# huzaifakhan04/truely-real-time-ai-generated-video-detection-framework-for-social-platforms

Hardware: AMD Instinct MI355X
Metric: frames/sec (detect+embed+drift) 720p (higher is better)
Workload: dtype f32; 1 GPU; BASELINE configs[1]: synthetic 720p 1-face frames, batch=256 per GPU, fp32, MTCNN detect + 80x80 crop + InceptionResnetV1 embed + cosine drift score; frames_per_gpu=256, height=720, width=1280, weights=seeded synthetic (no checkpoints offline), prelu_slopes=unit, min_face_size=20, pyramid_levels=11, valid_faces=256, score=6, emb_crc32=3015932725, mode=sharded, ingest=resident, parallelism=single GPU, batches_in_flight=1, driver=single, embed_group=8

## Files before the change

### truely-real-time-ai-generated-video-detection-framework-for-social-platforms_amd/csrc/trl_api.hip

```cpp
#include <limits.h>
#include <stdarg.h>
#include <stdio.h>
#include <string.h>
#include <stdlib.h>

#include "trl_ctx.h"

static thread_local char g_err[512] = "";
int g_trl_no_fnconv = 0;
int g_trl_pnet_gate = 0;

#include <mutex>
namespace {
std::mutex g_gate_mu;
hipEvent_t g_gate_ev[64] = {};
bool g_gate_set[64] = {};
}
int trl_gate_wait(trl_ctx* c, hipStream_t s) {
    const int d = c->cfg.device;
    if (!g_trl_pnet_gate || d < 0 || d >= 64) return TRL_OK;
    std::lock_guard<std::mutex> lk(g_gate_mu);
    if (g_gate_set[d]) TRL_HIP(hipStreamWaitEvent(s, g_gate_ev[d], 0));
    return TRL_OK;
}
// ... 856 lines not shown
    TRL_CHECK(check_crop_hook(c, d_frames, n, 65535, H, W, d_rect, d_valid, S, d_faces));
    return trl_launch_crop_area_std(d_frames, n, H, W, d_rect, d_valid, S, rgb != 0, d_faces, (hipStream_t)stream);
}
int trl_debug_nms_tiers(trl_ctx* c, int small_tier, int full_tier) {
    TRL_CHECK(trl_check_idle(c));
    if ((small_tier && (small_tier < 16 || small_tier > 3072 || (small_tier & 3))) || (full_tier && (full_tier < 16 || full_tier > 3072 || (full_tier & 3)))) {
        trl_set_error("tiers must be multiples of 4 in [16, 3072]");
        return TRL_ERR_INVALID;
    }
    if (small_tier) c->nms_small = small_tier;
    if (full_tier) c->nms_full = full_tier;
    return TRL_OK;
}
int trl_debug_list_stats(trl_ctx* c, long long* h_out8) {
    if (!c || !h_out8) { trl_set_error("null argument"); return TRL_ERR_INVALID; }
    const int32_t* f = c->h_pinned + 4;
    unsigned long long used = 0;
    memcpy(&used, f + FLG_SPILL_CUR, 8);
    int mx = 0;
    for (int l = 0; l < 32; l++) if (f[FLG_LEVEL_MAX + l] > mx) mx = f[FLG_LEVEL_MAX + l];
    h_out8[0] = c->last_attempts; h_out8[1] = f[FLG_SPILL_LISTS]; h_out8[2] = (long long)used; h_out8[3] = (long long)c->cb.spill_cap;
    h_out8[4] = c->cb.capF; h_out8[5] = c->cb.lay.S; h_out8[6] = mx; h_out8[7] = f[FLG_FRAME_MAX];
    return TRL_OK;
}

int trl_debug_option(trl_ctx* c, const char* key, int value) {
    if (!key) { trl_set_error("null key"); return TRL_ERR_INVALID; }
    if (!strcmp(key, "no_fnconv")) { g_trl_no_fnconv = value ? 1 : 0; return TRL_OK; }
    if (!strcmp(key, "pnet_gate")) { g_trl_pnet_gate = value ? 1 : 0; return TRL_OK; }
    TRL_CHECK(trl_check_idle(c));
    if (!strcmp(key, "rnet_chunk") && value >= 16) { c->rnet_chunk = value; return TRL_OK; }
    if (!strcmp(key, "onet_chunk") && value >= 16) { c->onet_chunk = value; return TRL_OK; }
    if (!strcmp(key, "pnet_screen") && (value == 0 || value == 1)) { c->pnet_screen = value; return TRL_OK; }
    trl_set_error("unknown option '%s' (or value %d out of range)", key, value);
    return TRL_ERR_INVALID;
}

int trl_debug_pnet_screen_bound(trl_ctx* c, float* A, float* B, int* on) {
    if (!c || !A || !B || !on) { trl_set_error("null argument"); return TRL_ERR_INVALID; }
    *A = c->pnet_scrA; *B = c->pnet_scrB; *on = c->pnet_screen_ok && c->pnet_screen;
    return TRL_OK;
}

int trl_debug_batch_capacity(trl_ctx* c, float t2_per_frame, float t3_per_frame, int* last_attempts) {
    if (!c) { trl_set_error("null context"); return TRL_ERR_INVALID; }
    if (t2_per_frame > 0.f) c->t2_per_frame = t2_per_frame;
    if (t3_per_frame > 0.f) c->t3_per_frame = t3_per_frame;
    if (last_attempts) *last_attempts = c->last_attempts;
    return TRL_OK;
}

int trl_debug_stage_totals(trl_ctx* c, int32_t* h_out2) {
    if (!c || !h_out2) { trl_set_error("null argument"); return TRL_ERR_INVALID; }
    h_out2[0] = c->h_pinned[4 + FLG_T2N]; h_out2[1] = c->h_pinned[4 + FLG_T3N];
    return TRL_OK;
}

int trl_debug_pnet_run(trl_ctx* c, int run) {
    if (!c || run < 0 || run > 64) { trl_set_error("bad argument"); return TRL_ERR_INVALID; }
    c->pnet_run = run;
    return TRL_OK;
}

int trl_debug_pnet_span(trl_ctx* c, int reset, double* ms_sum, int32_t* launches) {
    if (!c || !ms_sum || !launches) { trl_set_error("null argument"); return TRL_ERR_INVALID; }
    *ms_sum = 0.0; *launches = 0;
// ... 28 lines not shown
```

### truely-real-time-ai-generated-video-detection-framework-for-social-platforms_amd/csrc/trl_ctx.h

```cpp
#pragma once
#include "trl_common.h"

struct Cand {
    float x1, y1, x2, y2, score;
    float r0, r1, r2, r3;
    int cell;
};

struct LevelGeom {
    double scale;
    int h, w;
    int oh, ow;
};

struct LvLayout {
    int L = 0, S = 0;
    int capl[32] = {0}, rec0[32] = {0};
};
struct CascadeBufs {
    int n = 0, L = 0, H = 0, W = 0;
    LvLayout lay;
    int capF = 0;
    int32_t* lvl_cnt = nullptr;
    Cand* lvl_rec = nullptr;
// ... 33 lines not shown
    float last_ms[4] = {0, 0, 0, 0};
    int pnet_mono1 = 0;
    int pnet_unit = 0;
    float pnet_scrA = 0.f, pnet_scrB = 0.f;
    int pnet_screen_ok = 0;
    int pnet_screen = 1;
    int pnet_run = 0;
    int32_t* pnet_cursor = nullptr;
    unsigned long long* pnet_clk = nullptr;
    bool pnet_prof = false;
    float pnet_kernel_ms = 0.f;
    int dbg_poison = -1;
    float t2_per_frame = 160.f, t3_per_frame = 48.f;
    int cap_t2 = 0, cap_t3 = 0;
    float lvl_hint[32] = {0}, frame_hint = 0.f;
    size_t spill_hint = 0;
    int rnet_chunk = 49152, onet_chunk = 16384;
    int nms_small = 512, nms_full = 2048;
    int last_attempts = 0;
    int resume_stage = 0;
    size_t scratch_after_cascade = 0;
    int rnet_front_mode = -1, onet_front_mode = -1;
    struct Pending {
        enum Kind { EMBED, CROP, DETECT };
        bool active = false; int attempt = 0; Kind kind = EMBED;
        const uint8_t* frames = nullptr; int n = 0, H = 0, W = 0;
        void* stream = nullptr;
        float* box = nullptr; float* prob = nullptr; int32_t* rect = nullptr; uint8_t* valid = nullptr; float* emb = nullptr;
        float* faces_out = nullptr;
        float* boxes = nullptr; float* probs = nullptr; float* points = nullptr; int32_t* counts = nullptr; int order = 0;
    } pend;
    uint32_t* pyr_tab = nullptr;
    int pyr_tab_H = 0, pyr_tab_W = 0;
    struct { int nlev = 0, own0 = 0, band_cols = 0, strip_rows = 0, n_bands = 0, n_strips = 0; } pyr_fine;
    struct { int L = 0; int32_t row[16][TRL_PYR_PLAN_COLS] = {}; } pyr_plan;
    std::vector<trl_fn_plan_row> fn_plan;
    std::vector<trl_fn_plan_row> mt_plan;
    bool mt_plan_arm = false;
    int fn_cap_arm = -1;
    struct { void* p = nullptr; size_t cap = 0; int32_t dims[5] = {0, 0, 0, 0, 0}; } fn_cap[3];
};

struct TrlConvChoice { int family = 0, bm = 0, bn = 0, bk = 0, pad = 0, nz = 1; };
extern thread_local TrlConvChoice g_trl_conv_choice;

int trl_gate_wait(trl_ctx* c, hipStream_t s);
int trl_gate_record(trl_ctx* c, hipStream_t s);
extern int g_trl_pnet_gate;
int trl_ensure(trl_ctx* c, Arena& a, size_t bytes);
int trl_check_idle(trl_ctx* c);
const DevW* trl_w(trl_ctx* c, const std::string& name);
const DevV* trl_v(trl_ctx* c, const std::string& name);

int trl_run_facenet(trl_ctx* c, const float* d_faces, int n, int h, int w, const uint8_t* d_valid, float* d_emb, hipStream_t s);
int trl_run_rnet(trl_ctx* c, const float* d_crops, int n, float* d_out6, hipStream_t s);
int trl_run_onet(trl_ctx* c, const float* d_crops, int n, float* d_out16, hipStream_t s);
int trl_run_rnet_tail(trl_ctx* c, const float* d_pool1, int n, float* d_out6, hipStream_t s, const int32_t* n_dev = nullptr, int n_base = 0);
int trl_run_onet_tail(trl_ctx* c, const float* d_pool1, int n, float* d_out16, hipStream_t s, const int32_t* n_dev = nullptr, int n_base = 0);
int trl_launch_rnet_front(trl_ctx* c, const uint8_t* d_frames, int H, int W, const int32_t* d_total, int t0, int nc, float* d_pool, hipStream_t s);
int trl_launch_onet_front(trl_ctx* c, const uint8_t* d_frames, int H, int W, const int32_t* d_total, int t0, int nc, float* d_pool, hipStream_t s);
int trl_stage_net(trl_ctx* c, int net, const uint8_t* d_frames, int H, int W, const int32_t* d_total, int cap, float* d_out, hipStream_t s);
int trl_run_pnet_generic(trl_ctx* c, const float* d_level, int nf, int h, int w, float* d_heads, hipStream_t s);
size_t trl_pnet_generic_bytes(int nf, int h, int w);

int trl_cascade_detect(trl_ctx* c, const uint8_t* d_frames, int n, int H, int W, hipStream_t s, int resume = 0);
int trl_cascade_finish(trl_ctx* c, const uint8_t* d_frames, int n, int H, int W, float* d_boxes, float* d_probs, float* d_points,
// ... 24 lines not shown
```

### truely-real-time-ai-generated-video-detection-framework-for-social-platforms_amd/csrc/trl_pyramid.hip

```cpp
#include "trl_pyramid.h"
#include <type_traits>

typedef unsigned u32x4_a4 __attribute__((ext_vector_type(4), aligned(4)));
struct __attribute__((packed, aligned(4))) u32x3_a4 { unsigned x, y, z; };

namespace {

__device__ __forceinline__ void dword_sums(unsigned v, int rel, int nbytes, unsigned& s0, unsigned& s1, unsigned& s2) {
    const int lo = rel < 0 ? -rel : 0;
    const int hi = (nbytes - rel) < 4 ? (nbytes - rel) : 4;
    const unsigned vm = (hi >= 4 ? 0xFFFFFFFFu : ((1u << (8 * hi)) - 1u)) & ~((1u << (8 * lo)) - 1u);
    v &= vm;
    const int phase = (rel + 3) % 3;
    const unsigned m0 = phase == 0 ? 0x01000001u : (phase == 1 ? 0x00010000u : 0x00000100u);
    const unsigned m1 = phase == 0 ? 0x00000100u : (phase == 1 ? 0x01000001u : 0x00010000u);
    const unsigned m2 = phase == 0 ? 0x00010000u : (phase == 1 ? 0x00000100u : 0x01000001u);
    s0 = __builtin_amdgcn_udot4(v, m0, s0, false);
    s1 = __builtin_amdgcn_udot4(v, m1, s1, false);
    s2 = __builtin_amdgcn_udot4(v, m2, s2, false);
}

__device__ __forceinline__ unsigned chan_mask(int p, int c) {
    const int d = (c - p + 3) % 3;
    return d == 0 ? 0x01000001u : (d == 1 ? 0x00000100u : 0x00010000u);
}
__device__ __forceinline__ unsigned valid_bytes(int rel, int nbytes) {
    const int lo = rel < 0 ? -rel : 0;
    int hi = nbytes - rel; hi = hi < 0 ? 0 : (hi > 4 ? 4 : hi);
    if (lo >= hi) return 0u;
    return (hi >= 4 ? 0xFFFFFFFFu : ((1u << (8 * hi)) - 1u)) & ~((1u << (8 * lo)) - 1u);
}

typedef float f32x4_nt __attribute__((ext_vector_type(4)));
__device__ __forceinline__ void pyr_store(PyrPx* dst, const float4& v) {
    static_assert(sizeof(PyrPx) == 12, "layout");
    f32x3_nt t = {v.x, v.y, v.z};
    __builtin_nontemporal_store(t, reinterpret_cast<f32x3_nt*>(dst));
}

__device__ __forceinline__ float pyr_div(float a, float b, float r) {
    const float q0 = a * r;
    const float e = __builtin_fmaf(-b, q0, a);
    return __builtin_fmaf(e, r, q0);
}
__device__ __forceinline__ float pyr_norm(unsigned s, int kh, int kw, const PyrBins& g) {
    const float a = (float)s, fkh = (float)kh, fkw = (float)kw;
    float q;
    if (g.fastdiv) {
        const float r1 = kh == g.khA ? g.rkh[0] : g.rkh[1], r2 = kw == g.kwA ? g.rkw[0] : g.rkw[1];
        q = pyr_div(pyr_div(a, fkh, r1), fkw, r2);
    } else {
        q = a / fkh / fkw;
    }
    return (q - 127.5f) * 0.0078125f;
}

struct PyrArgs { int H, W, n_frames, f0; long long pyr_stride; PyrLevel g; };

template <int MODE>
__device__ __forceinline__ void pyr_level(const uint8_t* __restrict__ frames, const PyrArgs& a, const PyrLevel& g, const uint32_t* __restrict__ tab,
                                          PyrPx* __restrict__ pyr, int f, int q0, int qstep) {
    const int per_frame = g.pix_pad << g.gshift;
    constexpr int mode = MODE;
    const uint32_t* base32 = reinterpret_cast<const uint32_t*>(frames);
    const long long fbase = (long long)f * a.H * a.W * 3;
    const long long last_dw = ((long long)a.n_frames * a.H * a.W * 3 - 1) >> 2;
    const int row_bytes = a.W * 3;
    for (int q = q0; q < per_frame; q += qstep) {
        const int w = g.w, gsh = g.gshift, G = 1 << gsh;
        const int pixel = q >> gsh, sub = q & (G - 1);
        const bool valid = pixel < g.h * w;
        unsigned s0 = 0, s1 = 0, s2 = 0;
        int kh = 1, kw = 1;
        if (valid) {
            int oy = (int)__umulhi((unsigned)pixel, g.wmagic);
            oy -= (oy * w > pixel) ? 1 : 0;
// ... 274 lines not shown
                        c0 = n0; c1 = n1; c2 = n2; n0 = 0; n1 = 0; n2 = 0;
                        oy++;
                        ys_c = ys_n; ye_c = ye_n;
                        edges(oy + 1, ys_n, ye_n);
                    }
                }
            }
        }
    };
    if (lastf && yend >= a.H) run(std::true_type{}); else run(std::false_type{});
}

__global__ __launch_bounds__(192) void k_pyramid_fine(const uint8_t* __restrict__ frames, PyrFineArgs a, const uint32_t* __restrict__ tab,
                                                      PyrPx* __restrict__ pyr) {
    const int lane = threadIdx.x & 63, lvl = __builtin_amdgcn_readfirstlane((int)threadIdx.x >> 6);
    if (lvl >= a.nlev) return;
    const int band = blockIdx.x, strip = blockIdx.z, f = blockIdx.y;
    const uint32_t* own = tab + a.own0;
    const uint32_t cb = own[lvl * a.n_bands + band], rb = own[3 * a.n_bands + lvl * a.n_strips + strip];
    const int ox_lo = __builtin_amdgcn_readfirstlane((int)(cb & 0xFFFF)), ox_hi = __builtin_amdgcn_readfirstlane((int)(cb >> 16));
    const int oy_lo = __builtin_amdgcn_readfirstlane((int)(rb & 0xFFFF)), oy_hi = __builtin_amdgcn_readfirstlane((int)(rb >> 16));
    const bool pad_wave = band == 0 && strip == 0;
    if (lvl == 0) { if (a.g[0].kwmax * 3 + 3 > 16) pyr_fine_wave<true>(frames, a, a.g[0], tab, pyr, f, ox_lo, ox_hi, oy_lo, oy_hi, lane, pad_wave); else pyr_fine_wave<false>(frames, a, a.g[0], tab, pyr, f, ox_lo, ox_hi, oy_lo, oy_hi, lane, pad_wave); }
    else if (lvl == 1) { if (a.g[1].kwmax * 3 + 3 > 16) pyr_fine_wave<true>(frames, a, a.g[1], tab, pyr, f, ox_lo, ox_hi, oy_lo, oy_hi, lane, pad_wave); else pyr_fine_wave<false>(frames, a, a.g[1], tab, pyr, f, ox_lo, ox_hi, oy_lo, oy_hi, lane, pad_wave); }
    else { if (a.g[2].kwmax * 3 + 3 > 16) pyr_fine_wave<true>(frames, a, a.g[2], tab, pyr, f, ox_lo, ox_hi, oy_lo, oy_hi, lane, pad_wave); else pyr_fine_wave<false>(frames, a, a.g[2], tab, pyr, f, ox_lo, ox_hi, oy_lo, oy_hi, lane, pad_wave); }
}

constexpr int SMAXL = 12;
constexpr int SBYTES = 4096;
constexpr int SW_BYTES = 1280;
constexpr int STAB = 6144;
struct PyrStreamArgs {
    int H, W, n_frames, nlev, rows_per_band, cols_per_band, row_bands, col_bands;
    long long pyr_stride;
    PyrBins lv[SMAXL];
};

struct OwnBlock {
    static constexpr int LANES = 256, DW = 4, UNITS = 1, BYTES = SBYTES;
    static __device__ __forceinline__ int lane() { return threadIdx.x; }
    static __device__ __forceinline__ int slot() { return 0; }
    static __device__ __forceinline__ void sync() { __syncthreads(); }
    static __device__ __forceinline__ int uni(int x) { return x; }
};
struct OwnWave {
    static constexpr int LANES = 64, DW = 5, UNITS = 4, BYTES = SW_BYTES;
    static __device__ __forceinline__ int lane() { return threadIdx.x & 63; }
    static __device__ __forceinline__ int slot() { return __builtin_amdgcn_readfirstlane((int)threadIdx.x >> 6); }
    static __device__ __forceinline__ void sync() { __builtin_amdgcn_wave_barrier(); }
    static __device__ __forceinline__ int uni(int x) { return __builtin_amdgcn_readfirstlane(x); }
};

template <int NL, class Own>
__global__ __launch_bounds__(256) void k_pyramid_stream(const uint8_t* __restrict__ frames, PyrStreamArgs a, const uint32_t* __restrict__ gtab,
                                                        PyrPx* __restrict__ pyr) {
    constexpr int DW = Own::DW, LANES = Own::LANES;
    static_assert(Own::BYTES == 4 * DW * LANES && Own::UNITS * LANES == 256, "a lane's dwords tile the segment, the units the workgroup");
    __shared__ unsigned colbuf_all[Own::UNITS * Own::BYTES];
    __shared__ uint32_t tab[STAB];
    const int tid = threadIdx.x, lane = Own::lane(), slot = Own::slot();
    const int f = blockIdx.y;
    const int row_bytes = a.W * 3;
    const long long fbase = (long long)f * a.H * row_bytes;
    const long long last_dw = ((long long)a.n_frames * a.H * row_bytes - 1) >> 2;
    const uint32_t* base32 = reinterpret_cast<const uint32_t*>(frames);
    int ty0[NL], tx0[NL];
    {
        int pos = 0;
#pragma unroll
        for (int l = 0; l < NL; l++) {
            ty0[l] = tx0[l] = 0;
            if (l < a.nlev) {
                const PyrBins& g = a.lv[l];
                ty0[l] = pos; tx0[l] = pos + g.h;
                for (int i = tid; i < g.h; i += 256) tab[pos + i] = gtab[g.ytab0 + i];
                for (int i = tid; i < g.w; i += 256) tab[pos + g.h + i] = gtab[g.xtab0 + i];
                pos += g.h + g.w;
            }
        }
    }
    __syncthreads();
    const int unit = blockIdx.x * Own::UNITS + slot;
    if (Own::UNITS > 1 && unit >= a.row_bands * a.col_bands) return;
    const int rb = unit / a.col_bands, cb = unit - rb * a.col_bands;
    const int R0 = rb * a.rows_per_band, R1 = (R0 + a.rows_per_band < a.H) ? R0 + a.rows_per_band : a.H;
    const int C0 = cb * a.cols_per_band, C1 = (C0 + a.cols_per_band < a.W) ? C0 + a.cols_per_band : a.W;
    unsigned* colbuf = colbuf_all + slot * Own::BYTES;

    int j[NL], jend[NL], ys[NL], ye[NL], ox0[NL], ox1[NL];
    int yend = R0;
#pragma unroll
    for (int l = 0; l < NL; l++) {
        j[l] = jend[l] = 0; ys[l] = ye[l] = 0x7fffffff; ox0[l] = ox1[l] = 0;
        if (l < a.nlev) {
            const PyrBins& g = a.lv[l];
            auto first_at_or_after = [&](int tab0, int n_out, int n_in, int pos) {
                if (pos >= n_in) return n_out;
                int q = (int)(((long long)pos * n_out + n_in - 1) / n_in);
                if (q > n_out) q = n_out;
                while (q > 0 && (int)(tab[tab0 + q - 1] & 0xFFFF) >= pos) q--;
                while (q < n_out && (int)(tab[tab0 + q] & 0xFFFF) < pos) q++;
                return q;
            };
            j[l] = Own::uni(first_at_or_after(ty0[l], g.h, a.H, R0));
            jend[l] = Own::uni(first_at_or_after(ty0[l], g.h, a.H, R1));
            ox0[l] = Own::uni(first_at_or_after(tx0[l], g.w, a.W, C0));
            ox1[l] = Own::uni(first_at_or_after(tx0[l], g.w, a.W, C1));
            if (j[l] < jend[l] && ox0[l] < ox1[l]) {
                const uint32_t t0 = tab[ty0[l] + j[l]], t1 = tab[ty0[l] + jend[l] - 1];
                ys[l] = Own::uni((int)(t0 & 0xFFFF)); ye[l] = Own::uni((int)(t0 >> 16));
                const int e1 = Own::uni((int)(t1 >> 16));
                yend = e1 > yend ? e1 : yend;
            } else {
                j[l] = jend[l];
            }
        }
    }
    if (unit == 0) {
#pragma unroll
        for (int l = 0; l < NL; l++)
            if (l < a.nlev) {
                const PyrBins& g = a.lv[l];
                for (int p = g.h * g.w + lane; p < g.pix_pad; p += LANES)
                    pyr_store(pyr + ((long long)f * a.pyr_stride + g.pix0 + p), make_float4(0.f, 0.f, 0.f, 0.f));
            }
    }
    if (yend <= R0) return;

    unsigned ev[NL][DW], od[NL][DW];
#pragma unroll
    for (int l = 0; l < NL; l++)
#pragma unroll
        for (int d = 0; d < DW; d++) { ev[l][d] = 0; od[l][d] = 0; }

    auto load_row = [&](int y, unsigned (&w)[DW + 1], unsigned& sh) {
        const int yy = y < a.H ? y : a.H - 1;
        const long long o = fbase + (long long)yy * row_bytes + (long long)C0 * 3;
        sh = (unsigned)(o & 3);
        const long long dw = (o >> 2) + DW * lane;
        if (dw + DW <= last_dw) {
            const u32x4_a4 v4 = *reinterpret_cast<const u32x4_a4*>(base32 + dw);
            w[0] = v4[0]; w[1] = v4[1]; w[2] = v4[2]; w[3] = v4[3];
#pragma unroll
            for (int k = 4; k <= DW; k++) w[k] = base32[dw + k];
        } else {
#pragma unroll
            for (int k = 0; k <= DW; k++) w[k] = base32[dw + k <= last_dw ? dw + k : last_dw];
        }
    };
    auto consume = [&](int y, const unsigned (&w)[DW + 1], unsigned sh) {
        unsigned v[DW];
#pragma unroll
        for (int d = 0; d < DW; d++) v[d] = __builtin_amdgcn_alignbyte(w[d + 1], w[d], sh);
#pragma unroll
        for (int l = 0; l < NL; l++) {
            if (l < a.nlev && y >= ys[l] && y < ye[l]) {
#pragma unroll
                for (int d = 0; d < DW; d++) { ev[l][d] += v[d] & 0x00FF00FFu; od[l][d] += (v[d] >> 8) & 0x00FF00FFu; }
                if (y == ye[l] - 1) {
                    const PyrBins& g = a.lv[l];
                    const int kh = ye[l] - ys[l];
#pragma unroll
                    for (int d = 0; d < DW; d++) {
                        colbuf[4 * DW * lane + 4 * d + 0] = ev[l][d] & 0xFFFFu; colbuf[4 * DW * lane + 4 * d + 1] = od[l][d] & 0xFFFFu;
                        colbuf[4 * DW * lane + 4 * d + 2] = ev[l][d] >> 16;     colbuf[4 * DW * lane + 4 * d + 3] = od[l][d] >> 16;
                    }
                    Own::sync();
                    for (int ox = ox0[l] + lane; ox < ox1[l]; ox += LANES) {
                        const uint32_t tx = tab[tx0[l] + ox];
                        const int xs = tx & 0xFFFF, xe = tx >> 16;
                        unsigned s0 = 0, s1 = 0, s2 = 0;
                        for (int xx = xs; xx < xe; xx++) {
                            const unsigned* p = colbuf + (xx - C0) * 3;
                            s0 += p[0]; s1 += p[1]; s2 += p[2];
                        }
                        float4 o4;
                        o4.x = pyr_norm(s0, kh, xe - xs, g); o4.y = pyr_norm(s1, kh, xe - xs, g); o4.z = pyr_norm(s2, kh, xe - xs, g);
                        o4.w = 0.f;
                        pyr_store(pyr + ((long long)f * a.pyr_stride + g.pix0 + (long long)j[l] * g.w + ox), o4);
                    }
                    Own::sync();
                    j[l]++;
                    if (j[l] < jend[l]) {
                        const uint32_t t0 = tab[ty0[l] + j[l]];
                        ys[l] = Own::uni((int)(t0 & 0xFFFF)); ye[l] = Own::uni((int)(t0 >> 16));
                    } else {
                        ys[l] = ye[l] = 0x7fffffff;
                    }
                    const bool again = ys[l] <= y;
#pragma unroll
                    for (int d = 0; d < DW; d++) {
                        ev[l][d] = again ? (v[d] & 0x00FF00FFu) : 0u;
                        od[l][d] = again ? ((v[d] >> 8) & 0x00FF00FFu) : 0u;
                    }
                }
            }
        }
    };

    unsigned wb[4][DW + 1], shb[4];
#pragma unroll
    for (int u = 0; u < 4; u++) load_row(R0 + u, wb[u], shb[u]);
    for (int y = R0; y < yend; y += 4) {
#pragma unroll
        for (int u = 0; u < 4; u++) {
            unsigned wc[DW + 1];
#pragma unroll
            for (int k = 0; k <= DW; k++) wc[k] = wb[u][k];
            const unsigned shc = shb[u];
            if (y + u + 4 < yend) load_row(y + u + 4, wb[u], shb[u]);
            if (y + u < yend) consume(y + u, wc, shc);
        }
    }
}

}

int trl_pyramid_layout(trl_ctx* c, int H, int W, PyrLayout& lay) {
    const int L = trl_compute_levels(c, H, W);
    if (L > 16) { trl_set_error("more than 16 pyramid levels"); return TRL_ERR_INVALID; }
    if (L < 1) { trl_set_error("frame %dx%d has no pyramid level at min_face_size %d", W, H, c->cfg.min_face_size); return TRL_ERR_INVALID; }
    lay.L = L;
    int ntab = 0; long long pix = 0;
    for (int l = 0; l < L; l++) {
        const LevelGeom& g = c->lv[l];
        PyrLevel& p = lay.lv[l];
        p.h = g.h; p.w = g.w;
        p.pix0 = (int)pix;
        p.pix_pad = (int)(((long long)g.h * g.w + 63) & ~63ll);
        pix += p.pix_pad;
        const int khmax = (H + g.h - 1) / g.h + 1, kwmax = (W + g.w - 1) / g.w + 1;
        p.khA = (H + g.h - 1) / g.h; p.kwA = (W + g.w - 1) / g.w;
        p.khmax = (H % g.h) ? p.khA + 1 : p.khA; p.kwmax = (W % g.w) ? p.kwA + 1 : p.kwA;
        p.rkh[0] = 1.0f / (float)p.khA; p.rkh[1] = 1.0f / (float)(p.khA + 1);
        p.rkw[0] = 1.0f / (float)p.kwA; p.rkw[1] = 1.0f / (float)(p.kwA + 1);
        p.fastdiv = (p.khA + 1 <= 96 && p.kwA + 1 <= 96) ? 1 : 0;
        for (int d = 0; d < 4; d++) {
            auto vb = [](int rel, int nbytes) { int hi = nbytes - rel; hi = hi < 0 ? 0 : (hi > 4 ? 4 : hi); return hi >= 4 ? 0xFFFFFFFFu : ((1u << (8 * hi)) - 1u); };
            p.vmA[d] = vb(4 * d, 3 * p.kwA); p.vmB[d] = vb(4 * d, 3 * (p.kwA + 1));
        }
        p.wmagic = (unsigned)((0x100000000ull + g.w - 1) / g.w);
        p.hmagic = (unsigned)((0x100000000ull + g.h - 1) / g.h);
        p.arith = ((unsigned long long)(H + 1) * g.h * g.h < 0x100000000ull && (unsigned long long)(W + 1) * g.w * g.w < 0x100000000ull &&
                   g.h > 1 && g.w > 1) ? 1 : 0;
// ... 58 lines not shown
static int pyr_tables(trl_ctx* c, int H, int W, const PyrLayout& lay, hipStream_t s) {
    if (c->pyr_tab != nullptr && c->pyr_tab_H == H && c->pyr_tab_W == W) return TRL_OK;
    std::vector<uint32_t> tab;
    for (int l = 0; l < lay.L; l++) {
        const PyrLevel& g = lay.lv[l];
        for (int i = 0; i < g.h; i++) tab.push_back((uint32_t)(((long long)i * H) / g.h) | ((uint32_t)((((long long)i + 1) * H + g.h - 1) / g.h) << 16));
        for (int i = 0; i < g.w; i++) tab.push_back((uint32_t)(((long long)i * W) / g.w) | ((uint32_t)((((long long)i + 1) * W + g.w - 1) / g.w) << 16));
    }
    pyr_fine_ownership(c, H, W, lay, tab);
    TRL_HIP(hipStreamSynchronize(s));
    if (c->pyr_tab) TRL_HIP(hipFree(c->pyr_tab));
    c->pyr_tab = nullptr;
    TRL_HIP(hipMalloc((void**)&c->pyr_tab, tab.size() * 4 + 64));
    TRL_HIP(hipMemcpy(c->pyr_tab, tab.data(), tab.size() * 4, hipMemcpyHostToDevice));
    c->pyr_tab_H = H; c->pyr_tab_W = W;
    return TRL_OK;
}

struct PyrJob { trl_ctx* c; const uint8_t* frames; int n, H, W; const PyrLayout& lay; PyrPx* pyr; hipStream_t s; };
static void plan_row(const PyrJob& j, int l, int kind, int rb, int cb, int cpb, int frames) {
    int32_t* r = j.c->pyr_plan.row[l];
    r[0] = kind; r[1] = rb; r[2] = cb; r[3] = cpb; r[4] = frames; r[5] = j.lay.lv[l].khmax;
}

static int launch_coarse(const PyrJob& j, bool (&taken)[16]) {
    const int n = j.n, H = j.H, W = j.W;
    int lv_idx[16], nsel = 0;
    for (int l = 0; l < j.lay.L; l++) if (j.lay.lv[l].mode != 0) lv_idx[nsel++] = l;
    const bool wide = W * 3 > SBYTES;
    for (int g0 = 0; g0 < nsel; g0 += 8) {
        const int gn = nsel - g0 < 8 ? nsel - g0 : 8;
        PyrStreamArgs sa;
        sa.nlev = 0;
        int stab_words = 0, kwm = 0;
        bool ok = true;
        for (int q = 0; q < gn; q++) {
            const PyrLevel& g = j.lay.lv[lv_idx[g0 + q]];
            if (g.khmax > 256) ok = false;
            stab_words += g.h + g.w;
            kwm = g.kwmax > kwm ? g.kwmax : kwm;
            sa.lv[sa.nlev++] = g;
        }
        sa.H = H; sa.W = W; sa.n_frames = n; sa.pyr_stride = j.lay.pyr_stride;
        sa.row_bands = H >= 256 ? 3 : 1;
        sa.rows_per_band = (H + sa.row_bands - 1) / sa.row_bands;
        if (!ok || stab_words > STAB || n > 65535) continue;
        if (!wide) {
            if ((kwm + 2) * 3 > SBYTES / 2) continue;
            sa.col_bands = 1; sa.cols_per_band = W;
            const dim3 sgrid(sa.row_bands * sa.col_bands, n);
            if (sa.nlev <= 4) k_pyramid_stream<4, OwnBlock><<<sgrid, 256, 0, j.s>>>(j.frames, sa, j.c->pyr_tab, j.pyr);
            else k_pyramid_stream<8, OwnBlock><<<sgrid, 256, 0, j.s>>>(j.frames, sa, j.c->pyr_tab, j.pyr);
        } else {
            sa.cols_per_band = SW_BYTES / 3 - kwm;
            if (sa.cols_per_band < 64) continue;
            sa.col_bands = (W + sa.cols_per_band - 1) / sa.cols_per_band;
            sa.cols_per_band = (W + sa.col_bands - 1) / sa.col_bands;
            int rbn = (4096 + n * sa.col_bands - 1) / (n * sa.col_bands);
            if (rbn > H / 256) rbn = H / 256;
            if (rbn > sa.row_bands) { sa.row_bands = rbn; sa.rows_per_band = (H + rbn - 1) / rbn; }
            const dim3 sgrid((sa.row_bands * sa.col_bands + 3) / 4, n);
            if (sa.nlev <= 4) k_pyramid_stream<4, OwnWave><<<sgrid, 256, 0, j.s>>>(j.frames, sa, j.c->pyr_tab, j.pyr);
            else k_pyramid_stream<8, OwnWave><<<sgrid, 256, 0, j.s>>>(j.frames, sa, j.c->pyr_tab, j.pyr);
        }
        TRL_LAUNCH_CHECK();
        const int kind = wide ? (sa.nlev <= 4 ? TRL_PYR_SW4 : TRL_PYR_SW8) : (sa.nlev <= 4 ? TRL_PYR_S4 : TRL_PYR_S8);
        for (int q = 0; q < gn; q++) {
            taken[lv_idx[g0 + q]] = true;
            plan_row(j, lv_idx[g0 + q], kind, sa.row_bands, sa.col_bands, sa.cols_per_band, n);
        }
    }
    return TRL_OK;
}

static int launch_fine(const PyrJob& j, bool (&taken)[16]) {
    const auto& pf = j.c->pyr_fine;
    if (!(pf.nlev >= 2 && j.n <= 65535 && pf.n_strips <= 65535)) return TRL_OK;
    PyrFineArgs fa;
    fa.H = j.H; fa.W = j.W; fa.n_frames = j.n; fa.pyr_stride = j.lay.pyr_stride;
    fa.nlev = pf.nlev; fa.band_cols = pf.band_cols; fa.strip_rows = pf.strip_rows;
    fa.n_bands = pf.n_bands; fa.n_strips = pf.n_strips; fa.own0 = pf.own0;
    for (int l = 0; l < 3; l++) fa.g[l] = j.lay.lv[l < fa.nlev ? l : 0];
    k_pyramid_fine<<<dim3(fa.n_bands, j.n, fa.n_strips), 192, 0, j.s>>>(j.frames, fa, j.c->pyr_tab, j.pyr);
    TRL_LAUNCH_CHECK();
    for (int l = 0; l < fa.nlev; l++) { taken[l] = true; plan_row(j, l, TRL_PYR_FINE, 0, 0, 0, j.n); }
    return TRL_OK;
}

static int launch_per_level(const PyrJob& j, bool (&taken)[16]) {
    const int n = j.n;
    int chunk = (int)((176ll << 20) / ((long long)j.H * j.W * 3));
    if (chunk < 1) chunk = 1;
    if (chunk > n) chunk = n;
    for (int f0 = 0; f0 < n; f0 += chunk) {
        const int nf = (n - f0 < chunk) ? n - f0 : chunk;
        for (int l = 0; l < j.lay.L; l++) {
// ... 77 lines not shown
```

Baseline: 20570 frames/s.

## Restructure pyramid stream kernel with prefix sums, packed LDS strips and DPP reductions

Rewrites the coarse pyramid streaming kernel so each level's vertical box sum is taken as the difference of running 16-bit packed prefix sums, with level bookkeeping held in one lane per level and read via readlane and ballot. Column strips are stored as packed u16 in dynamic LDS and double-buffered for the 256-thread variant, which removes one barrier per output row. Horizontal sums split across sub-lanes and are combined with DPP adds. The table copy becomes a single contiguous range, and a debug option is added to force the number of row bands. The changes cut ALU work, LDS footprint and synchronisation, but prefix sums held in 16 bits may wrap and the tail-clamped loads add complexity.

```diff
diff --git a/truely-real-time-ai-generated-video-detection-framework-for-social-platforms_amd/csrc/trl_api.hip b/truely-real-time-ai-generated-video-detection-framework-for-social-platforms_amd/csrc/trl_api.hip
--- a/truely-real-time-ai-generated-video-detection-framework-for-social-platforms_amd/csrc/trl_api.hip
+++ b/truely-real-time-ai-generated-video-detection-framework-for-social-platforms_amd/csrc/trl_api.hip
@@ -912,6 +912,7 @@
     if (!strcmp(key, "rnet_chunk") && value >= 16) { c->rnet_chunk = value; return TRL_OK; }
     if (!strcmp(key, "onet_chunk") && value >= 16) { c->onet_chunk = value; return TRL_OK; }
     if (!strcmp(key, "pnet_screen") && (value == 0 || value == 1)) { c->pnet_screen = value; return TRL_OK; }
+    if (!strcmp(key, "pyr_row_bands") && value >= 0) { c->pyr_row_bands = value; return TRL_OK; }
     trl_set_error("unknown option '%s' (or value %d out of range)", key, value);
     return TRL_ERR_INVALID;
 }
diff --git a/truely-real-time-ai-generated-video-detection-framework-for-social-platforms_amd/csrc/trl_ctx.h b/truely-real-time-ai-generated-video-detection-framework-for-social-platforms_amd/csrc/trl_ctx.h
--- a/truely-real-time-ai-generated-video-detection-framework-for-social-platforms_amd/csrc/trl_ctx.h
+++ b/truely-real-time-ai-generated-video-detection-framework-for-social-platforms_amd/csrc/trl_ctx.h
@@ -89,6 +89,7 @@
     } pend;
     uint32_t* pyr_tab = nullptr;
     int pyr_tab_H = 0, pyr_tab_W = 0;
+    int pyr_row_bands = 0;
     struct { int nlev = 0, own0 = 0, band_cols = 0, strip_rows = 0, n_bands = 0, n_strips = 0; } pyr_fine;
     struct { int L = 0; int32_t row[16][TRL_PYR_PLAN_COLS] = {}; } pyr_plan;
     std::vector<trl_fn_plan_row> fn_plan;
diff --git a/truely-real-time-ai-generated-video-detection-framework-for-social-platforms_amd/csrc/trl_pyramid.hip b/truely-real-time-ai-generated-video-detection-framework-for-social-platforms_amd/csrc/trl_pyramid.hip
--- a/truely-real-time-ai-generated-video-detection-framework-for-social-platforms_amd/csrc/trl_pyramid.hip
+++ b/truely-real-time-ai-generated-video-detection-framework-for-social-platforms_amd/csrc/trl_pyramid.hip
@@ -3,6 +3,7 @@
 
 typedef unsigned u32x4_a4 __attribute__((ext_vector_type(4), aligned(4)));
 struct __attribute__((packed, aligned(4))) u32x3_a4 { unsigned x, y, z; };
+typedef unsigned short u16x2 __attribute__((ext_vector_type(2)));
 
 namespace {
 
@@ -42,6 +43,11 @@
     const float q0 = a * r;
     const float e = __builtin_fmaf(-b, q0, a);
     return __builtin_fmaf(e, r, q0);
+}
+__device__ __forceinline__ float pyr_norm(unsigned s, float fkh, float fkw, float r1, float r2, bool fast) {
+    const float a = (float)s;
+    const float q = fast ? pyr_div(pyr_div(a, fkh, r1), fkw, r2) : a / fkh / fkw;
+    return (q - 127.5f) * 0.0078125f;
 }
 __device__ __forceinline__ float pyr_norm(unsigned s, int kh, int kw, const PyrBins& g) {
     const float a = (float)s, fkh = (float)kh, fkw = (float)kw;
@@ -382,184 +388,235 @@
 constexpr int STAB = 6144;
 struct PyrStreamArgs {
     int H, W, n_frames, nlev, rows_per_band, cols_per_band, row_bands, col_bands;
+    int tab0, tab_words;
     long long pyr_stride;
     PyrBins lv[SMAXL];
 };
 
 struct OwnBlock {
-    static constexpr int LANES = 256, DW = 4, UNITS = 1, BYTES = SBYTES;
+    static constexpr int LANES = 256, DW = 4, UNITS = 1, BYTES = SBYTES, STRIPS = 2;
     static __device__ __forceinline__ int lane() { return threadIdx.x; }
     static __device__ __forceinline__ int slot() { return 0; }
     static __device__ __forceinline__ void sync() { __syncthreads(); }
-    static __device__ __forceinline__ int uni(int x) { return x; }
 };
 struct OwnWave {
-    static constexpr int LANES = 64, DW = 5, UNITS = 4, BYTES = SW_BYTES;
+    static constexpr int LANES = 64, DW = 5, UNITS = 4, BYTES = SW_BYTES, STRIPS = 1;
     static __device__ __forceinline__ int lane() { return threadIdx.x & 63; }
     static __device__ __forceinline__ int slot() { return __builtin_amdgcn_readfirstlane((int)threadIdx.x >> 6); }
     static __device__ __forceinline__ void sync() { __builtin_amdgcn_wave_barrier(); }
-    static __device__ __forceinline__ int uni(int x) { return __builtin_amdgcn_readfirstlane(x); }
 };
+
+extern __shared__ uint4 stream_lds[];
+template <class Own> constexpr int stream_strip_words() { return Own::UNITS * Own::STRIPS * Own::BYTES; }
+template <int CTRL> __device__ __forceinline__ unsigned dpp_add(unsigned s) {
+    return s + (unsigned)__builtin_amdgcn_update_dpp(0, (int)s, CTRL, 0xF, 0xF, false);
+}
 
 template <int NL, class Own>
 __global__ __launch_bounds__(256) void k_pyramid_stream(const uint8_t* __restrict__ frames, PyrStreamArgs a, const uint32_t* __restrict__ gtab,
                                                         PyrPx* __restrict__ pyr) {
     constexpr int DW = Own::DW, LANES = Own::LANES;
     static_assert(Own::BYTES == 4 * DW * LANES && Own::UNITS * LANES == 256, "a lane's dwords tile the segment, the units the workgroup");
-    __shared__ unsigned colbuf_all[Own::UNITS * Own::BYTES];
-    __shared__ uint32_t tab[STAB];
+    unsigned short* const strips = reinterpret_cast<unsigned short*>(stream_lds);
+    uint32_t* const tab = reinterpret_cast<uint32_t*>(strips + stream_strip_words<Own>());
     const int tid = threadIdx.x, lane = Own::lane(), slot = Own::slot();
     const int f = blockIdx.y;
     const int row_bytes = a.W * 3;
     const long long fbase = (long long)f * a.H * row_bytes;
     const long long last_dw = ((long long)a.n_frames * a.H * row_bytes - 1) >> 2;
     const uint32_t* base32 = reinterpret_cast<const uint32_t*>(frames);
-    int ty0[NL], tx0[NL];
-    {
-        int pos = 0;
-#pragma unroll
-        for (int l = 0; l < NL; l++) {
-            ty0[l] = tx0[l] = 0;
-            if (l < a.nlev) {
-                const PyrBins& g = a.lv[l];
-                ty0[l] = pos; tx0[l] = pos + g.h;
-                for (int i = tid; i < g.h; i += 256) tab[pos + i] = gtab[g.ytab0 + i];
-                for (int i = tid; i < g.w; i += 256) tab[pos + g.h + i] = gtab[g.xtab0 + i];
-                pos += g.h + g.w;
-            }
-        }
-    }
+    for (int i = tid; i < a.tab_words; i += 256) tab[i] = gtab[a.tab0 + i];
     __syncthreads();
     const int unit = blockIdx.x * Own::UNITS + slot;
     if (Own::UNITS > 1 && unit >= a.row_bands * a.col_bands) return;
     const int rb = unit / a.col_bands, cb = unit - rb * a.col_bands;
     const int R0 = rb * a.rows_per_band, R1 = (R0 + a.rows_per_band < a.H) ? R0 + a.rows_per_band : a.H;
     const int C0 = cb * a.cols_per_band, C1 = (C0 + a.cols_per_band < a.W) ? C0 + a.cols_per_band : a.W;
-    unsigned* colbuf = colbuf_all + slot * Own::BYTES;
-
-    int j[NL], jend[NL], ys[NL], ye[NL], ox0[NL], ox1[NL];
+    unsigned short* const colbuf = strips + slot * Own::STRIPS * Own::BYTES;
+    int flip = 0;
+
+    const int L = threadIdx.x & 63;
+    const bool has = L < a.nlev;
+    const PyrBins& gl = a.lv[has ? L : 0];
+    const int v_ty0 = gl.ytab0 - a.tab0, v_tx0 = gl.xtab0 - a.tab0, v_w = gl.w, v_pix0 = gl.pix0, v_khA = gl.khA, v_kwA = gl.kwA,
+              v_fast = gl.fastdiv;
+    const float v_rkh0 = gl.rkh[0], v_rkh1 = gl.rkh[1], v_rkw0 = gl.rkw[0], v_rkw1 = gl.rkw[1];
+    int v_j = 0, v_jend = 0, v_ys = 0x7fffffff, v_ye = 0x7fffffff, v_ox0 = 0, v_ox1 = 0, v_gs = 0, v_e1 = R0;
+    if (has) {
+        auto first_at_or_after = [&](int tab0, int n_out, int n_in, int pos) {
+            if (pos >= n_in) return n_out;
+            int q = (int)(((long long)pos * n_out + n_in - 1) / n_in);
+            if (q > n_out) q = n_out;
+            while (q > 0 && (int)(tab[tab0 + q - 1] & 0xFFFF) >= pos) q--;
+            while (q < n_out && (int)(tab[tab0 + q] & 0xFFFF) < pos) q++;
+            return q;
+        };
+        v_j = first_at_or_after(v_ty0, gl.h, a.H, R0);
+        v_jend = first_at_or_after(v_ty0, gl.h, a.H, R1);
+        v_ox0 = first_at_or_after(v_tx0, gl.w, a.W, C0);
+        v_ox1 = first_at_or_after(v_tx0, gl.w, a.W, C1);
+        while (v_gs < 4 && ((v_ox1 - v_ox0) << (v_gs + 1)) <= LANES && (2 << v_gs) <= gl.kwA) v_gs++;
+        if (v_j < v_jend && v_ox0 < v_ox1) {
+            const uint32_t t0 = tab[v_ty0 + v_j], t1 = tab[v_ty0 + v_jend - 1];
+            v_ys = (int)(t0 & 0xFFFF); v_ye = (int)(t0 >> 16);
+            v_e1 = (int)(t1 >> 16);
+        } else {
+            v_j = v_jend;
+        }
+    }
+    auto rl = [](int v, int l) { return __builtin_amdgcn_readlane(v, l); };
+    auto rlf = [](float v, int l) { return __builtin_bit_cast(float, __builtin_amdgcn_readlane(__builtin_bit_cast(int, v), l)); };
     int yend = R0;
-#pragma unroll
-    for (int l = 0; l < NL; l++) {
-        j[l] = jend[l] = 0; ys[l] = ye[l] = 0x7fffffff; ox0[l] = ox1[l] = 0;
-        if (l < a.nlev) {
+    for (int l = 0; l < a.nlev; l++) { const int e1 = rl(v_e1, l); yend = e1 > yend ? e1 : yend; }
+    if (unit == 0) {
+        for (int l = 0; l < a.nlev; l++) {
             const PyrBins& g = a.lv[l];
-            auto first_at_or_after = [&](int tab0, int n_out, int n_in, int pos) {
-                if (pos >= n_in) return n_out;
-                int q = (int)(((long long)pos * n_out + n_in - 1) / n_in);
-                if (q > n_out) q = n_out;
-                while (q > 0 && (int)(tab[tab0 + q - 1] & 0xFFFF) >= pos) q--;
-                while (q < n_out && (int)(tab[tab0 + q] & 0xFFFF) < pos) q++;
-                return q;
-            };
-            j[l] = Own::uni(first_at_or_after(ty0[l], g.h, a.H, R0));
-            jend[l] = Own::uni(first_at_or_after(ty0[l], g.h, a.H, R1));
-            ox0[l] = Own::uni(first_at_or_after(tx0[l], g.w, a.W, C0));
-            ox1[l] = Own::uni(first_at_or_after(tx0[l], g.w, a.W, C1));
-            if (j[l] < jend[l] && ox0[l] < ox1[l]) {
-                const uint32_t t0 = tab[ty0[l] + j[l]], t1 = tab[ty0[l] + jend[l] - 1];
-                ys[l] = Own::uni((int)(t0 & 0xFFFF)); ye[l] = Own::uni((int)(t0 >> 16));
-                const int e1 = Own::uni((int)(t1 >> 16));
-                yend = e1 > yend ? e1 : yend;
-            } else {
-                j[l] = jend[l];
-            }
-        }
-    }
-    if (unit == 0) {
-#pragma unroll
-        for (int l = 0; l < NL; l++)
-            if (l < a.nlev) {
-                const PyrBins& g = a.lv[l];
-                for (int p = g.h * g.w + lane; p < g.pix_pad; p += LANES)
-                    pyr_store(pyr + ((long long)f * a.pyr_stride + g.pix0 + p), make_float4(0.f, 0.f, 0.f, 0.f));
-            }
+            for (int p = g.h * g.w + lane; p < g.pix_pad; p += LANES)
+                pyr_store(pyr + ((long long)f * a.pyr_stride + g.pix0 + p), make_float4(0.f, 0.f, 0.f, 0.f));
+        }
     }
     if (yend <= R0) return;
 
-    unsigned ev[NL][DW], od[NL][DW];
+    u16x2 pe[DW], po[DW], se[NL][DW], so[NL][DW];
+#pragma unroll
+    for (int d = 0; d < DW; d++) { pe[d] = 0; po[d] = 0; }
 #pragma unroll
     for (int l = 0; l < NL; l++)
 #pragma unroll
-        for (int d = 0; d < DW; d++) { ev[l][d] = 0; od[l][d] = 0; }
-
+        for (int d = 0; d < DW; d++) { se[l][d] = 0; so[l][d] = 0; }
+
+    const long long lim_dw = last_dw - DW > 0 ? last_dw - DW : 0;
     auto load_row = [&](int y, unsigned (&w)[DW + 1], unsigned& sh) {
         const int yy = y < a.H ? y : a.H - 1;
         const long long o = fbase + (long long)yy * row_bytes + (long long)C0 * 3;
         sh = (unsigned)(o & 3);
-        const long long dw = (o >> 2) + DW * lane;
-        if (dw + DW <= last_dw) {
-            const u32x4_a4 v4 = *reinterpret_cast<const u32x4_a4*>(base32 + dw);
-            w[0] = v4[0]; w[1] = v4[1]; w[2] = v4[2]; w[3] = v4[3];
-#pragma unroll
-            for (int k = 4; k <= DW; k++) w[k] = base32[dw + k];
-        } else {
-#pragma unroll
-            for (int k = 0; k <= DW; k++) w[k] = base32[dw + k <= last_dw ? dw + k : last_dw];
-        }
-    };
-    auto consume = [&](int y, const unsigned (&w)[DW + 1], unsigned sh) {
-        unsigned v[DW];
-#pragma unroll
-        for (int d = 0; d < DW; d++) v[d] = __builtin_amdgcn_alignbyte(w[d + 1], w[d], sh);
-#pragma unroll
-        for (int l = 0; l < NL; l++) {
-            if (l < a.nlev && y >= ys[l] && y < ye[l]) {
-#pragma unroll
-                for (int d = 0; d < DW; d++) { ev[l][d] += v[d] & 0x00FF00FFu; od[l][d] += (v[d] >> 8) & 0x00FF00FFu; }
-                if (y == ye[l] - 1) {
-                    const PyrBins& g = a.lv[l];
-                    const int kh = ye[l] - ys[l];
-#pragma unroll
-                    for (int d = 0; d < DW; d++) {
-                        colbuf[4 * DW * lane + 4 * d + 0] = ev[l][d] & 0xFFFFu; colbuf[4 * DW * lane + 4 * d + 1] = od[l][d] & 0xFFFFu;
-                        colbuf[4 * DW * lane + 4 * d + 2] = ev[l][d] >> 16;     colbuf[4 * DW * lane + 4 * d + 3] = od[l][d] >> 16;
+        long long dw = (o >> 2) + DW * lane;
+        dw = dw < lim_dw ? dw : lim_dw;
+        const u32x4_a4 v4 = *reinterpret_cast<const u32x4_a4*>(base32 + dw);
+        w[0] = v4[0]; w[1] = v4[1]; w[2] = v4[2]; w[3] = v4[3];
+#pragma unroll
+        for (int k = 4; k <= DW; k++) w[k] = base32[dw + k];
+    };
+    auto fix_tail = [&](int y, unsigned (&w)[DW + 1]) {
+        const int yy = y < a.H ? y : a.H - 1;
+        const long long dw0 = (fbase + (long long)yy * row_bytes + (long long)C0 * 3) >> 2;
+        if (dw0 + DW * (LANES - 1) <= lim_dw) return;
+        const long long over = dw0 + DW * lane - lim_dw;
+#pragma unroll
+        for (int m = 1; m <= DW; m++)
+            if (over == m) {
+#pragma unroll
+                for (int k = 0; k + m <= DW; k++) w[k] = w[k + m];
+            }
+    };
+    auto unpack = [&](int y, unsigned (&w)[DW + 1], unsigned sh, u16x2 (&re)[DW], u16x2 (&ro)[DW]) {
+        fix_tail(y, w);
+#pragma unroll
+        for (int d = 0; d < DW; d++) {
+            const unsigned v = __builtin_amdgcn_alignbyte(w[d + 1], w[d], sh);
+            re[d] = __builtin_bit_cast(u16x2, v & 0x00FF00FFu); ro[d] = __builtin_bit_cast(u16x2, (v >> 8) & 0x00FF00FFu);
+        }
+    };
+    auto consume = [&](int y, const u16x2 (&re)[DW], const u16x2 (&ro)[DW]) {
+        const unsigned starts = (unsigned)__builtin_amdgcn_ballot_w64(v_ys == y);
+        const unsigned ends = (unsigned)__builtin_amdgcn_ballot_w64(v_ye == y + 1);
+        if (starts) {
+#pragma unroll
+            for (int l = 0; l < NL; l++)
+                if (starts >> l & 1) {
+#pragma unroll
+                    for (int d = 0; d < DW; d++) { se[l][d] = pe[d]; so[l][d] = po[d]; }
+                }
+        }
+#pragma unroll
+        for (int d = 0; d < DW; d++) { pe[d] += re[d]; po[d] += ro[d]; }
+        for (unsigned m = ends; m; m &= m - 1) {
+            const int l = __builtin_ctz(m);
+            u16x2 ce[DW], co[DW];
+#pragma unroll
+            for (int k = 0; k < NL; k++)
+                if (l == k) {
+#pragma unroll
+                    for (int d = 0; d < DW; d++) { ce[d] = pe[d] - se[k][d]; co[d] = po[d] - so[k][d]; }
+                }
+            const int jl = rl(v_j, l), kh = rl(v_ye, l) - rl(v_ys, l), ox0 = rl(v_ox0, l), ox1 = rl(v_ox1, l), gsh = rl(v_gs, l);
+            const int ty0 = rl(v_ty0, l), tx0 = rl(v_tx0, l), kwA = rl(v_kwA, l);
+            const float fkh = (float)kh, rh = kh == rl(v_khA, l) ? rlf(v_rkh0, l) : rlf(v_rkh1, l), rw0 = rlf(v_rkw0, l), rw1 = rlf(v_rkw1, l);
+            const bool fast = rl(v_fast, l) != 0;
+            PyrPx* const orow = pyr + ((long long)f * a.pyr_stride + rl(v_pix0, l) + (long long)jl * rl(v_w, l));
+            unsigned short* const strip = colbuf + flip * Own::BYTES;
+            uint2* const dst = reinterpret_cast<uint2*>(strip + 4 * DW * lane);
+#pragma unroll
+            for (int d = 0; d < DW; d++) dst[d] = make_uint2(ce[d].x | ((unsigned)co[d].x << 16), ce[d].y | ((unsigned)co[d].y << 16));
+            Own::sync();
+            const int nth = (ox1 - ox0) << gsh;
+            for (int t = lane; t < nth; t += LANES) {
+                const int ox = ox0 + (t >> gsh), sub = t & ((1 << gsh) - 1);
+                const uint32_t tx = tab[tx0 + ox];
+                const int xs = tx & 0xFFFF, xe = tx >> 16;
+                unsigned s0 = 0, s1 = 0, s2 = 0;
+                for (int x0 = xs + sub; x0 < xe; x0 += 4 << gsh) {
+                    unsigned q[4][3];
+#pragma unroll
+                    for (int k = 0; k < 4; k++) {
+                        const int xx = x0 + (k << gsh);
+                        const unsigned short* p = strip + ((xx < xe ? xx : x0) - C0) * 3;
+                        q[k][0] = p[0]; q[k][1] = p[1]; q[k][2] = p[2];
                     }
-                    Own::sync();
-                    for (int ox = ox0[l] + lane; ox < ox1[l]; ox += LANES) {
-                        const uint32_t tx = tab[tx0[l] + ox];
-                        const int xs = tx & 0xFFFF, xe = tx >> 16;
-                        unsigned s0 = 0, s1 = 0, s2 = 0;
-                        for (int xx = xs; xx < xe; xx++) {
-                            const unsigned* p = colbuf + (xx - C0) * 3;
-                            s0 += p[0]; s1 += p[1]; s2 += p[2];
-                        }
-                        float4 o4;
-                        o4.x = pyr_norm(s0, kh, xe - xs, g); o4.y = pyr_norm(s1, kh, xe - xs, g); o4.z = pyr_norm(s2, kh, xe - xs, g);
-                        o4.w = 0.f;
-                        pyr_store(pyr + ((long long)f * a.pyr_stride + g.pix0 + (long long)j[l] * g.w + ox), o4);
-                    }
-                    Own::sync();
-                    j[l]++;
-                    if (j[l] < jend[l]) {
-                        const uint32_t t0 = tab[ty0[l] + j[l]];
-                        ys[l] = Own::uni((int)(t0 & 0xFFFF)); ye[l] = Own::uni((int)(t0 >> 16));
-                    } else {
-                        ys[l] = ye[l] = 0x7fffffff;
-                    }
-                    const bool again = ys[l] <= y;
-#pragma unroll
-                    for (int d = 0; d < DW; d++) {
-                        ev[l][d] = again ? (v[d] & 0x00FF00FFu) : 0u;
-                        od[l][d] = again ? ((v[d] >> 8) & 0x00FF00FFu) : 0u;
+#pragma unroll
+                    for (int k = 0; k < 4; k++) {
+                        const bool in = x0 + (k << gsh) < xe;
+                        s0 += in ? q[k][0] : 0u; s1 += in ? q[k][1] : 0u; s2 += in ? q[k][2] : 0u;
                     }
                 }
-            }
-        }
-    };
-
-    unsigned wb[4][DW + 1], shb[4];
-#pragma unroll
-    for (int u = 0; u < 4; u++) load_row(R0 + u, wb[u], shb[u]);
-    for (int y = R0; y < yend; y += 4) {
-#pragma unroll
-        for (int u = 0; u < 4; u++) {
-            unsigned wc[DW + 1];
-#pragma unroll
-            for (int k = 0; k <= DW; k++) wc[k] = wb[u][k];
-            const unsigned shc = shb[u];
-            if (y + u + 4 < yend) load_row(y + u + 4, wb[u], shb[u]);
-            if (y + u < yend) consume(y + u, wc, shc);
+                if (gsh > 0) { s0 = dpp_add<0xB1>(s0); s1 = dpp_add<0xB1>(s1); s2 = dpp_add<0xB1>(s2); }
+                if (gsh > 1) { s0 = dpp_add<0x4E>(s0); s1 = dpp_add<0x4E>(s1); s2 = dpp_add<0x4E>(s2); }
+                if (gsh > 2) { s0 = dpp_add<0x141>(s0); s1 = dpp_add<0x141>(s1); s2 = dpp_add<0x141>(s2); }
+                if (gsh > 3) { s0 = dpp_add<0x140>(s0); s1 = dpp_add<0x140>(s1); s2 = dpp_add<0x140>(s2); }
+                if (sub == 0) {
+                    const float fkw = (float)(xe - xs), rw = xe - xs == kwA ? rw0 : rw1;
+                    float4 o4;
+                    o4.x = pyr_norm(s0, fkh, fkw, rh, rw, fast); o4.y = pyr_norm(s1, fkh, fkw, rh, rw, fast);
+                    o4.z = pyr_norm(s2, fkh, fkw, rh, rw, fast); o4.w = 0.f;
+                    pyr_store(orow + ox, o4);
+                }
+            }
+            if (Own::STRIPS > 1) flip ^= 1; else Own::sync();
+            int nys = 0x7fffffff, nye = 0x7fffffff;
+            if (jl + 1 < rl(v_jend, l)) {
+                const uint32_t t0 = tab[ty0 + jl + 1];
+                nys = __builtin_amdgcn_readfirstlane((int)(t0 & 0xFFFF)); nye = __builtin_amdgcn_readfirstlane((int)(t0 >> 16));
+            }
+            if (L == l) { v_j = jl + 1; v_ys = nys; v_ye = nye; }
+            if (nys <= y) {
+#pragma unroll
+                for (int k = 0; k < NL; k++)
+                    if (l == k) {
+#pragma unroll
+                        for (int d = 0; d < DW; d++) { se[k][d] = pe[d] - re[d]; so[k][d] = po[d] - ro[d]; }
+                    }
+            }
+        }
+    };
+
+    constexpr int PF = 2;
+    unsigned wb[PF][DW + 1], shb[PF], wn[PF][DW + 1], shn[PF];
+#pragma unroll
+    for (int u = 0; u < PF; u++) load_row(R0 + u, wb[u], shb[u]);
+    for (int y = R0; y < yend; y += PF) {
+#pragma unroll
+        for (int u = 0; u < PF; u++) load_row(y + PF + u, wn[u], shn[u]);
+#pragma unroll
+        for (int u = 0; u < PF; u++) {
+            u16x2 re[DW], ro[DW];
+            unpack(y + u, wb[u], shb[u], re, ro);
+            if (y + u < yend) consume(y + u, re, ro);
+        }
+#pragma unroll
+        for (int u = 0; u < PF; u++) {
+#pragma unroll
+            for (int k = 0; k <= DW; k++) wb[u][k] = wn[u][k];
+            shb[u] = shn[u];
         }
     }
 }
@@ -684,25 +741,31 @@
         const int gn = nsel - g0 < 8 ? nsel - g0 : 8;
         PyrStreamArgs sa;
         sa.nlev = 0;
-        int stab_words = 0, kwm = 0;
+        int tab_lo = 0x7fffffff, tab_hi = 0, kwm = 0;
         bool ok = true;
         for (int q = 0; q < gn; q++) {
             const PyrLevel& g = j.lay.lv[lv_idx[g0 + q]];
             if (g.khmax > 256) ok = false;
-            stab_words += g.h + g.w;
+            tab_lo = g.ytab0 < tab_lo ? g.ytab0 : tab_lo;
+            tab_hi = g.xtab0 + g.w > tab_hi ? g.xtab0 + g.w : tab_hi;
             kwm = g.kwmax > kwm ? g.kwmax : kwm;
             sa.lv[sa.nlev++] = g;
         }
+        const int stab_words = tab_hi - tab_lo;
+        sa.tab0 = tab_lo; sa.tab_words = stab_words;
         sa.H = H; sa.W = W; sa.n_frames = n; sa.pyr_stride = j.lay.pyr_stride;
-        sa.row_bands = H >= 256 ? 3 : 1;
+        const int forced = j.c->pyr_row_bands;
+        sa.row_bands = forced > 0 ? (forced < H ? forced : H) : (H >= 256 ? 3 : 1);
         sa.rows_per_band = (H + sa.row_bands - 1) / sa.row_bands;
+        sa.row_bands = (H + sa.rows_per_band - 1) / sa.rows_per_band;
         if (!ok || stab_words > STAB || n > 65535) continue;
         if (!wide) {
             if ((kwm + 2) * 3 > SBYTES / 2) continue;
             sa.col_bands = 1; sa.cols_per_band = W;
             const dim3 sgrid(sa.row_bands * sa.col_bands, n);
-            if (sa.nlev <= 4) k_pyramid_stream<4, OwnBlock><<<sgrid, 256, 0, j.s>>>(j.frames, sa, j.c->pyr_tab, j.pyr);
-            else k_pyramid_stream<8, OwnBlock><<<sgrid, 256, 0, j.s>>>(j.frames, sa, j.c->pyr_tab, j.pyr);
+            const size_t lds = stream_strip_words<OwnBlock>() * 2 + (size_t)stab_words * 4;
+            if (sa.nlev <= 4) k_pyramid_stream<4, OwnBlock><<<sgrid, 256, lds, j.s>>>(j.frames, sa, j.c->pyr_tab, j.pyr);
+            else k_pyramid_stream<8, OwnBlock><<<sgrid, 256, lds, j.s>>>(j.frames, sa, j.c->pyr_tab, j.pyr);
         } else {
             sa.cols_per_band = SW_BYTES / 3 - kwm;
             if (sa.cols_per_band < 64) continue;
@@ -710,10 +773,11 @@
             sa.cols_per_band = (W + sa.col_bands - 1) / sa.col_bands;
             int rbn = (4096 + n * sa.col_bands - 1) / (n * sa.col_bands);
             if (rbn > H / 256) rbn = H / 256;
-            if (rbn > sa.row_bands) { sa.row_bands = rbn; sa.rows_per_band = (H + rbn - 1) / rbn; }
+            if (rbn > sa.row_bands && forced <= 0) { sa.row_bands = rbn; sa.rows_per_band = (H + rbn - 1) / rbn; }
             const dim3 sgrid((sa.row_bands * sa.col_bands + 3) / 4, n);
-            if (sa.nlev <= 4) k_pyramid_stream<4, OwnWave><<<sgrid, 256, 0, j.s>>>(j.frames, sa, j.c->pyr_tab, j.pyr);
-            else k_pyramid_stream<8, OwnWave><<<sgrid, 256, 0, j.s>>>(j.frames, sa, j.c->pyr_tab, j.pyr);
+            const size_t lds = stream_strip_words<OwnWave>() * 2 + (size_t)stab_words * 4;
+            if (sa.nlev <= 4) k_pyramid_stream<4, OwnWave><<<sgrid, 256, lds, j.s>>>(j.frames, sa, j.c->pyr_tab, j.pyr);
+            else k_pyramid_stream<8, OwnWave><<<sgrid, 256, lds, j.s>>>(j.frames, sa, j.c->pyr_tab, j.pyr);
         }
         TRL_LAUNCH_CHECK();
         const int kind = wide ? (sa.nlev <= 4 ? TRL_PYR_SW4 : TRL_PYR_SW8) : (sa.nlev <= 4 ? TRL_PYR_S4 : TRL_PYR_S8);
```

Result: faster. 20980 frames/s (median of 6 runs) (+2.0%).
